# NVIDIA/cuopt

Measured on NVIDIA H100. Metric: pdlp_iterations_per_sec, higher is better.
Workload: dtype f64

## Files before the change

### cuopt_b200/csrc/pdlp_kernels.cuh

```cuda
#pragma once

#include "device_utils.cuh"
#include "spmv_bicsr.cuh"

#include <math_constants.h>

namespace cuopt_b200 {

constexpr int EW_THREADS  = 256;
static __device__ int g_l2_hints = 1;

struct pdhg_ctl_t {
  double step_size, primal_weight, tau, sigma;
  double pending_weight;
  double sum_weights;
  double interaction, norm_dx2, norm_dy2;
  double reduction_exponent, growth_exponent, primal_smoothing, dual_smoothing;
  int parity;
  int pending_avg;
  int active;
  int valid;
  int k_pdhg;
  int attempts;
  int accepted;
// ... 90 lines not shown
constexpr int DIST_MAX_PEERS        = 8;
constexpr int DIST_FLAG_XBAR        = 0 * DIST_MAX_PEERS;
constexpr int DIST_FLAG_Y           = 1 * DIST_MAX_PEERS;
constexpr int DIST_FLAG_SCALARS     = 2 * DIST_MAX_PEERS;
constexpr int DIST_FLAG_XBAR_B      = 3 * DIST_MAX_PEERS;
constexpr int DIST_FLAG_Y_B         = 4 * DIST_MAX_PEERS;
constexpr int DIST_FLAG_COUNT       = 5 * DIST_MAX_PEERS;
constexpr long long DIST_SPIN_LIMIT = 20000000000LL;
struct peer_ptrs_t {
  double* p[DIST_MAX_PEERS];
};
struct peer_flags_t {
  unsigned long long* p[DIST_MAX_PEERS];
};
__device__ __forceinline__ void st_release_sys(unsigned long long* p, unsigned long long v)
{
  asm volatile("st.release.sys.global.u64 [%0], %1;" ::"l"(p), "l"(v) : "memory");
}
__device__ __forceinline__ unsigned long long ld_acquire_sys(const unsigned long long* p)
{
  unsigned long long v;
  asm volatile("ld.acquire.sys.global.u64 %0, [%1];" : "=l"(v) : "l"(p) : "memory");
  return v;
}
__device__ __forceinline__ void peer_wait(const unsigned long long* flags, int count, unsigned long long epoch)
{
  if ((int)threadIdx.x < count) {
    const long long t0 = clock64();
    while (ld_acquire_sys(flags + threadIdx.x) < epoch) {
      __nanosleep(64);
      if (clock64() - t0 > DIST_SPIN_LIMIT) __trap();
    }
  }
  __syncthreads();
}
__device__ __forceinline__ void peer_signal_grid_done(unsigned* ticket, const peer_flags_t& flags, int world, int index,
                                                      unsigned long long epoch, int index2 = -1)
{
  __threadfence_system();
  __syncthreads();
  if (threadIdx.x != 0) return;
  const unsigned t = atomicAdd(ticket, 1u);
  if (t != gridDim.x - 1) return;
  *ticket = 0u;
  __threadfence_system();
#pragma unroll
  for (int r = 0; r < DIST_MAX_PEERS; ++r)
    if (r < world) {
      st_release_sys(flags.p[r] + index, epoch);
      if (index2 >= 0) st_release_sys(flags.p[r] + index2, epoch);
    }
}

__global__ void __launch_bounds__(EW_THREADS) k_primal_step(const pdhg_ctl_t* __restrict__ ctl,
                                                            int n,
                                                            double* __restrict__ xbuf0,
                                                            double* __restrict__ xbuf1,
                                                            const double* __restrict__ aty0,
                                                            const double* __restrict__ aty1,
                                                            const double* __restrict__ c,
                                                            const double* __restrict__ l,
                                                            const double* __restrict__ u,
                                                            double* __restrict__ sum_x,
                                                            double* __restrict__ xbar)
{
  if (!ctl->active) return;
  const int cur           = ctl->parity;
  const double* x         = cur ? xbuf1 : xbuf0;
  double* xn              = cur ? xbuf0 : xbuf1;
  const double* aty       = cur ? aty1 : aty0;
  const double tau        = ctl->tau;
  const bool pending      = ctl->pending_avg != 0;
  const double w          = ctl->pending_weight;
  const int stride        = gridDim.x * blockDim.x;
  const l2_policy_t pol   = make_l2_policies(g_l2_hints);
  for (int j = blockIdx.x * blockDim.x + threadIdx.x; j < n; j += stride) {
    const double xj = x[j];
    if (pending) sum_x[j] = sum_x[j] + w * xj;
    const double gradient = ld_stream(c + j) - aty[j];
    double next           = xj - (tau * gradient);
    next                  = fmax(fmin(next, ld_stream(u + j)), ld_stream(l + j));
    xn[j]                 = next;
    st_l2(xbar + j, next - xj + next, pol.keep);
  }
}

template <bool INIT, int NPRE, bool BCAST = false>
__global__ void __launch_bounds__(BICSR_THREADS, bicsr_min_ctas(NPRE)) k_dual_step(pdhg_ctl_t* __restrict__ ctl,
                                                                             bicsr_view_t A,
                                                                             const double* __restrict__ xbar,
                                                                             double* __restrict__ ybuf0,
                                                                             double* __restrict__ ybuf1,
                                                                             const double* __restrict__ lc,
                                                                             const double* __restrict__ uc,
                                                                             double* __restrict__ sum_y,
                                                                             double* __restrict__ part_dy2,
                                                                             const unsigned long long* xbar_flags,
                                                                             int n_xbar_flags,
                                                                             const double* __restrict__ t,
                                                                             peer_ptrs_t y_peers = peer_ptrs_t{},
                                                                             peer_flags_t flags = peer_flags_t{},
                                                                             int world = 1,
                                                                             int rank = 0,
                                                                             const int* __restrict__ send = nullptr,
                                                                             int send_stride = 0)
{
  if (!ctl->active) return;
  __shared__ double rows[BICSR_WARPS][BICSR_SLOTS];
  __shared__ double red[32];
  const unsigned long long epoch = (unsigned long long)ctl->attempts + 1ull;
  if (xbar_flags) peer_wait(xbar_flags, n_xbar_flags, (unsigned long long)ctl->attempts + 1ull);
  const int cur      = ctl->parity;
  const double* y    = cur ? ybuf1 : ybuf0;
  double* yn         = cur ? ybuf0 : ybuf1;
  const double sigma = ctl->sigma;
  const bool pending = ctl->pending_avg != 0;
  const double w     = ctl->pending_weight;
  double dy2         = 0.0;
  const l2_policy_t pol = make_l2_policies(g_l2_hints);
  struct payload_t {
    double y, lc, uc, sum, init;
  };
  auto pre_op = [&](int i) {
    payload_t p;
    p.y    = y[i];
    p.lc   = ld_stream(lc + i);
    p.uc   = ld_stream(uc + i);
    p.sum  = pending ? sum_y[i] : 0.0;
    p.init = INIT ? ld_l2(t + i, pol.stream) : 0.0;
    return p;
  };
  auto row_op = [&](int i, double s, const payload_t& p) {
    if (pending) sum_y[i] = p.sum + w * p.y;
    double next      = p.y - (sigma * s);
    const double low = next + sigma * p.lc;
    const double up  = next + sigma * p.uc;
    next             = fmax(low, fmin(up, 0.0));
    st_l2(yn + i, next, pol.keep);
    if constexpr (BCAST) {
#pragma unroll
      for (int r = 0; r < DIST_MAX_PEERS; ++r)
        if (r < world) {
          const int d = __ldg(send + (size_t)r * send_stride + i);
          if (d >= 0) y_peers.p[r][d] = next;
        }
    }
    const double d   = next - p.y;
    dy2 += d * d;
  };
  spmv_bicsr_rows<payload_t, INIT, NPRE>(A, xbar, rows[threadIdx.x >> 5], pre_op, row_op, pol.keep);
  const double tot = block_reduce(dy2, red);
  if (threadIdx.x == 0) part_dy2[blockIdx.x] = tot;
  if constexpr (BCAST) peer_signal_grid_done(&ctl->ticket[2], flags, world, DIST_FLAG_Y + rank, epoch, DIST_FLAG_Y_B + rank);
}

template <bool INIT, int NPRE>
__global__ void __launch_bounds__(BICSR_THREADS, bicsr_min_ctas(NPRE)) k_transpose_step(pdhg_ctl_t* __restrict__ ctl,
                                                                                  bicsr_view_t AT,
                                                                                  const double* __restrict__ ybuf0,
                                                                                  const double* __restrict__ ybuf1,
                                                                                  const double* __restrict__ xbuf0,
                                                                                  const double* __restrict__ xbuf1,
                                                                                  double* __restrict__ aty0,
                                                                                  double* __restrict__ aty1,
                                                                                  double* __restrict__ parts,
                                                                                  const double* __restrict__ part_dy2,
                                                                                  int n_part_dy2,
                                                                                  const double* __restrict__ t)
{
// ... 338 lines not shown
                                                                  int nloc,
                                                                  const double* __restrict__ src,
                                                                  const double* __restrict__ xbuf0,
                                                                  const double* __restrict__ xbuf1,
                                                                  double* __restrict__ aty0,
                                                                  double* __restrict__ aty1,
                                                                  double* __restrict__ parts,
                                                                  const double* __restrict__ part_dy2,
                                                                  int n_part_dy2,
                                                                  double* __restrict__ scal)
{
  if (!ctl->active) return;
  __shared__ double red[32];
  const int cur     = ctl->parity;
  const double* x   = cur ? xbuf1 : xbuf0;
  const double* xn  = cur ? xbuf0 : xbuf1;
  const double* aty = cur ? aty1 : aty0;
  double* atyn      = cur ? aty0 : aty1;
  double acc[2]     = {0.0, 0.0};
  const int stride  = gridDim.x * blockDim.x;
  for (int j = blockIdx.x * blockDim.x + threadIdx.x; j < nloc; j += stride) {
    double s = 0.0;
    s += __ldcg(src + j);
    atyn[j]        = s;
    const double d = xn[j] - x[j];
    acc[0] += d * (s - aty[j]);
    acc[1] += d * d;
  }
  if (!publish_and_elect<2>(acc, parts, &ctl->ticket[0], red)) return;
  const double interaction = gather_partials(parts, gridDim.x, red);
  const double dx2         = gather_partials(parts + gridDim.x, gridDim.x, red);
  const double dy2         = gather_partials(part_dy2, n_part_dy2, red);
  if (threadIdx.x != 0) return;
  scal[0] = interaction;
  scal[1] = dx2;
  scal[2] = dy2;
}

__global__ void k_step_rule_gather(pdhg_ctl_t* __restrict__ ctl, const double* __restrict__ scal, int n_src,
                                   const unsigned long long* wait_flags)
{
  if (!ctl->active) return;
  if (wait_flags) peer_wait(wait_flags, n_src, (unsigned long long)ctl->attempts + 1ull);
  if (threadIdx.x != 0) return;
  double interaction = 0.0, dx2 = 0.0, dy2 = 0.0;
  for (int g = 0; g < n_src; ++g) {
    interaction += __ldcg(scal + 4 * g + 0);
    dx2 += __ldcg(scal + 4 * g + 1);
    dy2 += __ldcg(scal + 4 * g + 2);
  }
  pdhg_step_rule(ctl, interaction, dx2, dy2);
}

__global__ void __launch_bounds__(BICSR_THREADS, BICSR_MIN_CTAS) k_block_pass(const pdhg_ctl_t* __restrict__ ctl,
                                                                              bicsr_view_t Ab,
                                                                              const double* __restrict__ x0,
                                                                              const double* __restrict__ x1,
                                                                              int pick_candidate,
                                                                              double* __restrict__ t,
                                                                              int first,
                                                                              const unsigned long long* wait_flags,
                                                                              int n_wait)
{
  if (!ctl->active) return;
  __shared__ double rows[BICSR_WARPS][BICSR_SLOTS];
  if (wait_flags) peer_wait(wait_flags, n_wait, (unsigned long long)ctl->attempts + 1ull);
  const double* x       = pick_candidate ? (ctl->parity ? x0 : x1) : x0;
  const l2_policy_t pol = make_l2_policies(g_l2_hints);
  struct payload_t {
    double init;
  };
  auto pre_op = [&](int r) {
    payload_t p;
    p.init = first ? 0.0 : ld_l2(t + r, pol.stream);
    return p;
  };
  auto row_op = [&](int r, double s, const payload_t&) { st_l2(t + r, s, pol.stream); };
  spmv_bicsr_rows<payload_t, true>(Ab, x, rows[threadIdx.x >> 5], pre_op, row_op, pol.keep);
}

__global__ void __launch_bounds__(EW_THREADS) k_flush_average(const pdhg_ctl_t* __restrict__ ctl,
                                                              int n,
                                                              const double* __restrict__ xbuf0,
                                                              const double* __restrict__ xbuf1,
                                                              double* __restrict__ sum_x,
                                                              int m,
                                                              const double* __restrict__ ybuf0,
                                                              const double* __restrict__ ybuf1,
                                                              double* __restrict__ sum_y)
{
  if (!ctl->pending_avg) return;
  const int cur    = ctl->parity;
  const double* x  = cur ? xbuf1 : xbuf0;
  const double* y  = cur ? ybuf1 : ybuf0;
  const double w   = ctl->pending_weight;
  const int stride = gridDim.x * blockDim.x;
  for (int j = blockIdx.x * blockDim.x + threadIdx.x; j < n; j += stride) sum_x[j] = sum_x[j] + w * x[j];
  for (int i = blockIdx.x * blockDim.x + threadIdx.x; i < m; i += stride) sum_y[i] = sum_y[i] + w * y[i];
}
__global__ void k_clear_pending(pdhg_ctl_t* ctl) { ctl->pending_avg = 0; }
__global__ void k_begin_batch(pdhg_ctl_t* ctl, int steps)
{
  ctl->target = ctl->accepted + steps;
  ctl->valid  = 0;
  ctl->active = steps > 0 ? 1 : 0;
}

__global__ void __launch_bounds__(BICSR_THREADS, BICSR_MIN_CTAS) k_spmv(bicsr_view_t A,
                                                                        const double* __restrict__ x,
                                                                        double* __restrict__ out)
{
  __shared__ double rows[BICSR_WARPS][BICSR_SLOTS];
  struct payload_t {};
  auto pre_op = [&](int) { return payload_t{}; };
  auto row_op = [&](int i, double s, const payload_t&) { out[i] = s; };
  spmv_bicsr_rows<payload_t>(A, x, rows[threadIdx.x >> 5], pre_op, row_op, make_l2_policies(g_l2_hints).keep);
}

__global__ void __launch_bounds__(BICSR_THREADS, BICSR_MIN_CTAS) k_spmv_pair(bicsr_view_t M,
                                                                             const double* __restrict__ u,
                                                                             const double* __restrict__ v,
                                                                             double* __restrict__ out_u,
                                                                             double* __restrict__ out_v,
                                                                             int first)
{
  __shared__ double rows[2][BICSR_WARPS][BICSR_SLOTS];
  auto row_op = [&](int r, double su, double sv) {
    out_u[r] = first ? su : out_u[r] + su;
    out_v[r] = first ? sv : out_v[r] + sv;
  };
  const int w = threadIdx.x >> 5;
// ... 541 lines not shown
```

### cuopt_b200/csrc/pdlp_solver.cu

```cuda
#include "pdlp_solver.hpp"

#include "dist_comm.hpp"
#include "pdlp_kernels.cuh"
#include "trust_region.cuh"

#include <math_constants.h>
#include <nvtx3/nvToolsExt.h>

#include <algorithm>
#include <chrono>
#include <cmath>
#include <cstdio>
#include <cstdlib>
#include <atomic>
#include <map>
#include <mutex>
#include <thread>
#include <string>

namespace cuopt_b200 {

namespace {

struct bicsr_dev_t {
// ... 310 lines not shown
    cudaEventSynchronize(tr_ev[last]);
    for (int i = 0; i < last; ++i) {
      float ms = 0.f;
      cudaEventElapsedTime(&ms, tr_ev[i], tr_ev[i + 1]);
      tr_acc[i] += ms;
    }
    ++tr_count;
  }
  int nslice = 0, n_pad = 0, slice_j0 = 0, slice_n = 0, grid_slice = 1;
  dvec<double> rs_buf, scal;
  dvec<unsigned long long> d_flags;
  void* xbar_peer[DIST_MAX_PEERS]  = {};
  void* scal_peer[DIST_MAX_PEERS]  = {};
  void* flag_peer[DIST_MAX_PEERS]  = {};
  bool peers_open = false;
  peer_ptrs_t p_xbar{}, p_scal{};
  peer_flags_t p_flags{};
  dvec<unsigned> d_ticket;
  dvec<pdhg_ctl_t> d_ctl;
  dvec<eval_t> d_eval;
  pdhg_ctl_t* h_ctl = nullptr;
  eval_t* h_eval    = nullptr;
  double* h_scalar  = nullptr;
  int occ_spmv = 1;
  int occ_spmv2 = 1;
  int npre_override = 0;
  dvec<double> eval_m, eval_n;
  dvec<double> part_max;
  dvec<double> part_infeas;
  bool tr_enabled = false;
  double tr_gap_reduction_last_trial = 1.0;
  int grid_tr = 1;
  dvec<double> tr_aty, tr_ax, tr_grad, tr_dir, tr_thr, tr_thr_sorted, tr_A, tr_B, tr_parts, tr_scal;
  dvec<int> tr_iota, tr_perm;
  struct tr_gap_t {
    const double *px, *py;
    double pd = 0, dd = 0, dist = 0, lower = 0, upper = 0, ngap = 0;
  };
  struct gather_blocks_t {
    int B = 1, width = 0;
    std::vector<csr_dev_t> blk;
    std::vector<csr_dev_t> unscaled;
    std::vector<int> grid;
    bool on() const { return B > 1; }
  };
  gather_blocks_t blkA, blkAT, blkATslice;
  dvec<double> t_m, t_n;
  size_t gather_block_bytes = 0;
  int n_part_dy2 = 1;
  int grid_k1 = 1, grid_k2 = 1, grid_k3 = 1, grid_n = 1, grid_m = 1, grid_misc = 1;
  long long staged_fills = 0;
  std::map<int, cudaGraphExec_t> graphs;
  bool use_graphs = true;
  cudaEvent_t ev_a = nullptr, ev_b = nullptr;

  int total_pdlp_iterations      = 0;
  bool initialised               = false;
  bool need_aty                  = true;
  bool last_restart_was_average  = false;
  bool warm_started              = false;
  double last_candidate_kkt      = 0.0, last_restart_kkt = 0.0;
  double l2_norm_b = 0.0, l2_norm_c = 0.0;
  lp_solution_t sol;
  bool finished   = false;
  double t_start  = 0.0;
  long long launches = 0;

  void close_peer_memory(bool collective)
  {
    if (!peers_open) return;
    cudaStreamSynchronize(stream);
    dist->close_peers(xbar_peer);
    dist->close_peers(scal_peer);
    dist->close_peers(flag_peer);
    dist->close_peers(yfull_peer);
    peers_open = false;
    if (collective) {
      dist->allreduce(d_scalar.data(), 1, true, stream);
      cudaStreamSynchronize(stream);
    }
  }

  ~impl_t()
  {
    if (trace.on) {
      const alloc_stats_t& a = alloc_stats();
      std::fprintf(stderr, "[cuopt-b200 trace] so far in this process: %ld cudaMalloc %.1f ms (%.2f GB), %ld cudaFree %.1f ms\n",
                   a.n_malloc, 1e3 * a.malloc_s, a.bytes * 1e-9, a.n_free, 1e3 * a.free_s);
    }
    if (dist_trace && tr_count > 0)
      std::fprintf(stderr, "[cuopt-b200 dist trace] rank %d of %d, gather transport, %ld attempts: K1 %.1f us, K2 %.1f us, K3 %.1f us, rule %.1f us "
                   "(each slot includes the wait for the peers' flags)\n", dist->rank, dist->world, tr_count,
                   1e3 * tr_acc[0] / tr_count, 1e3 * tr_acc[1] / tr_count, 1e3 * tr_acc[2] / tr_count, 1e3 * tr_acc[3] / tr_count);
    for (auto& e : tr_ev) if (e) cudaEventDestroy(e);
    if (ev_fork) cudaEventDestroy(ev_fork);
    if (ev_join) cudaEventDestroy(ev_join);
    if (comm_stream) cudaStreamDestroy(comm_stream);
    close_peer_memory(false);
    for (auto& g : graphs) cudaGraphExecDestroy(g.second);
    if (ev_a) cudaEventDestroy(ev_a);
    if (ev_b) cudaEventDestroy(ev_b);
    if (h_ctl) cudaFreeHost(h_ctl);
    if (h_eval) cudaFreeHost(h_eval);
    if (h_scalar) cudaFreeHost(h_scalar);
    if (stream) cudaStreamDestroy(stream);
  }

  int spmv_grid(const csr_dev_t& M, int npre = 1) const
  {
    const int reserve = (dist_gather && dist_send_kernel) ? send_slots : 0;
    const int wave    = std::max(1, sms * (npre > 1 ? occ_spmv2 : occ_spmv) - reserve);
    return std::max(1, std::min((M.n_blk() + BICSR_WARPS - 1) / BICSR_WARPS, wave));
  }
  int fused_npre(const csr_dev_t& M) const
  {
    if (npre_override) return npre_override > 1 ? 2 : 1;
    const bicsr_dev_t& b = M.bi_structure();
    return (b.n_std > 0 && (long long)M.rows > 40LL * b.n_std) ? 2 : 1;
  }

  void sync() { CUOPT_CUDA_TRY(cudaStreamSynchronize(stream)); }
  void check_launch() { CUOPT_CUDA_TRY(cudaGetLastError()); }

  phase_trace_t trace;
  void build(const lp_problem_t& p, const pdlp_settings_t& settings)
  {
    nvtx_range_t nvtx_scope("pdlp build: upload, transpose, block-interleaved matrices");
    trace.start(nullptr);
    p.check_representation();
    trace.mark("check_representation");
    st       = settings;
    hp       = pdlp_hyper_params_t::preset(settings.pdlp_solver_mode);
    m        = p.n_constraints;
    n        = p.n_variables;
    nnz      = p.nnz();
    maximize = p.maximize;
    if (m == 0 || nnz == 0) {
      throw lp_error(error_type_t::Success, "No constraints in the problem: PDLP can't be run");
    }
    int dev = 0;
    CUOPT_CUDA_TRY(cudaGetDevice(&dev));
    CUOPT_CUDA_TRY(cudaDeviceGetAttribute(&sms, cudaDevAttrMultiProcessorCount, dev));
    CUOPT_CUDA_TRY(cudaStreamCreateWithFlags(&stream, cudaStreamNonBlocking));
    CUOPT_CUDA_TRY(cudaEventCreate(&ev_a));
    CUOPT_CUDA_TRY(cudaEventCreate(&ev_b));
    CUOPT_CUDA_TRY(cudaMallocHost(&h_ctl, sizeof(pdhg_ctl_t)));
    CUOPT_CUDA_TRY(cudaMallocHost(&h_eval, 2 * sizeof(eval_t)));
    CUOPT_CUDA_TRY(cudaMallocHost(&h_scalar, 8 * sizeof(double)));
    if (const char* e = std::getenv("CUOPT_B200_NO_GRAPH")) use_graphs = !(e[0] == '1');
    if (const char* e = std::getenv("CUOPT_B200_L2_HINTS")) {
      const int on = e[0] != '0';
      CUOPT_CUDA_TRY(cudaMemcpyToSymbol(g_l2_hints, &on, sizeof(int)));
    }

    obj_scale  = p.objective_scaling_factor;
    obj_offset = p.objective_offset;
    if (maximize) obj_scale = -obj_scale;
    trace.stream = stream;
    trace.mark("stream + pinned control buffers");
    const long long fills0 = staged_uploader_t::get().fills();
    upload_csr(A, m, n, p.A_offsets, p.A_indices, p.A_values, stream, sms);
    trace.mark("upload A + BICSR(A)");
    transpose_to(AT, A, stream, sms);
    trace.mark("transpose + BICSR(A^T)");
    As.alias_structure_copy_values(A, stream);
    ATs.alias_structure_copy_values(AT, stream);
    const int gn = ew_grid(n, sms), gm = ew_grid(m, sms);
    upload_staged(c, p.objective_coefficients, stream);
    if (maximize) k_scale_constant<<<gn, EW_THREADS, 0, stream>>>(n, c.data(), -1.0);
    if (p.variable_lower_bounds.empty()) {
      l.resize(n);
      k_fill<<<gn, EW_THREADS, 0, stream>>>(n, l.data(), 0.0);
    } else {
      upload_staged(l, p.variable_lower_bounds, stream);
    }
    if (p.variable_upper_bounds.empty()) {
      u.resize(n);
      k_fill<<<gn, EW_THREADS, 0, stream>>>(n, u.data(), std::numeric_limits<double>::infinity());
    } else {
      upload_staged(u, p.variable_upper_bounds, stream);
    }
    if (!p.constraint_lower_bounds.empty()) {
      upload_staged(lc, p.constraint_lower_bounds, stream);
      upload_staged(uc, p.constraint_upper_bounds, stream);
    } else {
      hvec<double> hlc, huc;
      p.row_bounds(hlc, huc);
      upload_staged(lc, hlc, stream);
      upload_staged(uc, huc, stream);
      sync();
    }
    {
      dvec<int> bad(2);
      bad.zero(stream);
      k_count_crossed_bounds<<<gn, EW_THREADS, 0, stream>>>(n, l.data(), u.data(), bad.data());
      k_count_crossed_bounds<<<gm, EW_THREADS, 0, stream>>>(m, lc.data(), uc.data(), bad.data() + 1);
      check_launch();
      int h_bad[2] = {0, 0};
      CUOPT_CUDA_TRY(cudaMemcpyAsync(h_bad, bad.data(), sizeof(h_bad), cudaMemcpyDeviceToHost, stream));
      sync();
      if (h_bad[0]) throw lp_error(error_type_t::ValidationError, "Variable lower bound above upper bound");
      if (h_bad[1]) throw lp_error(error_type_t::ValidationError, "Constraint lower bound above upper bound");
// ... 550 lines not shown
      g.blk[b].cols = M.cols;
      g.blk[b].off.resize((size_t)M.rows + 1);
      offs[b] = g.blk[b].off.data();
    }
    csr_split_columns_offsets(M.rows, M.off_ptr(), M.idx_ptr(), g.width, B, offs.data(), nnz_b.data(), stream);
    for (int b = 0; b < B; ++b) {
      g.blk[b].nnz = nnz_b[b];
      g.blk[b].idx.resize((size_t)nnz_b[b]);
      g.blk[b].val.resize((size_t)nnz_b[b]);
      idxs[b] = g.blk[b].idx.data();
      vals[b] = g.blk[b].val.data();
    }
    csr_split_columns_fill(M.rows, M.off_ptr(), M.idx_ptr(), M.val.data(), g.width, B, offs.data(), idxs.data(), vals.data(),
                           stream);
    std::vector<int> hoff((size_t)M.rows + 1);
    g.grid.resize(B);
    for (int b = 0; b < B; ++b) {
      g.blk[b].off.download(hoff.data(), stream);
      sync();
      build_bicsr(g.blk[b], hoff, stream, sms);
      g.grid[b] = spmv_grid(g.blk[b]);
    }
    if (unscaled_src) {
      g.unscaled.resize(B);
      for (int b = 0; b < B; ++b) {
        csr_dev_t& U = g.unscaled[b];
        U.rows = M.rows; U.cols = M.cols; U.nnz = nnz_b[b];
        U.structure = &g.blk[b];
        U.val.resize((size_t)nnz_b[b]);
        vals[b] = U.val.data();
      }
      csr_split_columns_fill(M.rows, M.off_ptr(), M.idx_ptr(), unscaled_src->val.data(), g.width, B, offs.data(), idxs.data(),
                             vals.data(), stream);
      for (csr_dev_t& U : g.unscaled) {
        fill_bicsr_values(U, stream, sms);
        if (U.bi_structure().n_std == U.bi_structure().n_blk) {
          sync();
          U.val = dvec<double>{};
        }
      }
    }
    t.resize((size_t)M.rows);
    t.zero(stream);
  }
  void launch_block_passes(const gather_blocks_t& g, int count, const double* x0, const double* x1, int pick_candidate,
                           double* t, const unsigned long long* wait_flags, int n_wait)
  {
    for (int b = 0; b < count; ++b) {
      const csr_dev_t& M = g.blk[b];
      k_block_pass<<<g.grid[b], BICSR_THREADS, 0, stream>>>(d_ctl.data(), M.view(), x0, x1, pick_candidate, t, b == 0,
                                                            b == 0 ? wait_flags : nullptr, n_wait);
    }
  }
  void enqueue_k2(const unsigned long long* wait_flags, int n_wait, bool bcast = false,
                  const unsigned long long* wait_flags_b = nullptr)
  {
    const bool blocked  = blkA.on();
    const csr_dev_t& L  = blocked ? blkA.blk[blkA.B - 1] : hot_A();
    const int npre      = fused_npre(L);
    const int grid      = spmv_grid(L, npre);
    const double* t     = blocked ? t_m.data() : nullptr;
    const unsigned long long* wf = wait_flags_b ? wait_flags_b : (blocked ? nullptr : wait_flags);
    if (blocked) launch_block_passes(blkA, blkA.B - 1, xbar.data(), xbar.data(), 0, t_m.data(), wait_flags, n_wait);
#define CUOPT_K2(INIT, NPRE)                                                                                             \
  k_dual_step<INIT, NPRE><<<grid, BICSR_THREADS, 0, stream>>>(d_ctl.data(), L.view(), xbar.data(), ybuf[0].data(),       \
                                                              ybuf[1].data(), lcs.data(), ucs.data(), sum_y.data(),      \
                                                              part_dy2.data(), wf, n_wait, t)
#define CUOPT_K2B(INIT, NPRE)                                                                                            \
  k_dual_step<INIT, NPRE, true><<<grid, BICSR_THREADS, 0, stream>>>(d_ctl.data(), L.view(), xbar.data(), ybuf[0].data(), \
                                                                    ybuf[1].data(), lcs.data(), ucs.data(), sum_y.data(), \
                                                                    part_dy2.data(), wf, n_wait, t, p_yfull, p_flags,     \
                                                                    dist->world, dist->rank, sendY.data(), m)
    if (bcast) {
      if (blocked) { if (npre > 1) CUOPT_K2B(true, 2); else CUOPT_K2B(true, 1); }
      else { if (npre > 1) CUOPT_K2B(false, 2); else CUOPT_K2B(false, 1); }
    } else if (blocked) { if (npre > 1) CUOPT_K2(true, 2); else CUOPT_K2(true, 1); }
    else { if (npre > 1) CUOPT_K2(false, 2); else CUOPT_K2(false, 1); }
#undef CUOPT_K2B
#undef CUOPT_K2
  }
  int k2_grid() const
  {
    const csr_dev_t& L = blkA.on() ? blkA.blk[blkA.B - 1] : hot_A();
    return spmv_grid(L, fused_npre(L));
  }
  int k3_npre() const { return npre_override > 1 ? 2 : 1; }
  int k3_grid() const { return spmv_grid(blkAT.on() ? blkAT.blk[blkAT.B - 1] : ATs, k3_npre()); }
  void enqueue_k3()
  {
    const bool blocked = blkAT.on();
    const csr_dev_t& L = blocked ? blkAT.blk[blkAT.B - 1] : ATs;
    const int npre     = k3_npre();
    const int grid     = k3_grid();
    const double* t    = blocked ? t_n.data() : nullptr;
    if (blocked) launch_block_passes(blkAT, blkAT.B - 1, ybuf[0].data(), ybuf[1].data(), 1, t_n.data(), nullptr, 0);
#define CUOPT_K3(INIT, NPRE)                                                                                              \
  k_transpose_step<INIT, NPRE><<<grid, BICSR_THREADS, 0, stream>>>(d_ctl.data(), L.view(), ybuf[0].data(), ybuf[1].data(), \
                                                                   xbuf[0].data(), xbuf[1].data(), atybuf[0].data(),      \
                                                                   atybuf[1].data(), part_k3.data(), part_dy2.data(),     \
                                                                   n_part_dy2, t)
    if (blocked) { if (npre > 1) CUOPT_K3(true, 2); else CUOPT_K3(true, 1); }
    else { if (npre > 1) CUOPT_K3(false, 2); else CUOPT_K3(false, 1); }
#undef CUOPT_K3
  }
  int kernels_per_attempt() const
  {
    const int k2 = blkA.on() ? blkA.B : 1;
    if (!sharded()) return 1 + k2 + (blkAT.on() ? blkAT.B : 1);
    if (dist_gather) return 1 + k2 + (blkATslice.on() ? blkATslice.B : 1) + 1 + (dist_send_kernel ? 2 : 0);
    return 1 + k2 + (blkAT.on() ? blkAT.B : 1) + 2;
  }

  void launch_transpose_partial()
  {
    if (blkAT.on()) {
      launch_block_passes(blkAT, blkAT.B, ybuf[0].data(), ybuf[1].data(), 1, dist_buf.data(), nullptr, 0);
      return;
    }
    k_transpose_partial<<<grid_k3, BICSR_THREADS, 0, stream>>>(d_ctl.data(), ATs.view(), ybuf[0].data(), ybuf[1].data(),
                                                               dist_buf.data());
  }
  void launch_spmv(const csr_dev_t& M, const double* v, double* out)
  {
    k_spmv<<<spmv_grid(M), BICSR_THREADS, 0, stream>>>(M.view(), v, out);
  }
  int launch_spmv_pair(const csr_dev_t& M, const gather_blocks_t& g, const double* u, const double* v, double* out_u,
                       double* out_v)
  {
    const int count = g.unscaled.empty() ? 1 : (int)g.unscaled.size();
    for (int b = 0; b < count; ++b) {
// ... 21 lines not shown
      } else {
        k_primal_step_bcast<<<grid_slice, EW_THREADS, 0, stream>>>(d_ctl.data(), slice_n, x0, x1, a0, a1, cs.data() + j0,
                                                                   ls.data() + j0, us.data() + j0, sum_x.data() + j0, p_xbar,
                                                                   p_flags, G, rk, sendX.data(), nslice);
      }
      tr_tick(1);
      enqueue_k2(fl + DIST_FLAG_XBAR, G, !dist_send_kernel, fl + DIST_FLAG_XBAR_B);
      tr_tick(2);
      if (dist_send_kernel) {
        CUOPT_CUDA_TRY(cudaEventRecord(ev_fork, stream));
        CUOPT_CUDA_TRY(cudaStreamWaitEvent(comm_stream, ev_fork, 0));
        k_send_packed<<<grid_send, EW_THREADS, 0, comm_stream>>>(d_ctl.data(), ybuf[0].data(), ybuf[1].data(), 1, listY.data(),
                                                                 sendY.data(), m, planY, p_yfull, p_flags, G, rk,
                                                                 DIST_FLAG_Y, DIST_FLAG_Y_B, d_ticket.data() + 4);
        CUOPT_CUDA_TRY(cudaEventRecord(ev_join, comm_stream));
      }
      const bool blocked = blkATslice.on();
      const csr_dev_t& L = blocked ? blkATslice.blk[blkATslice.B - 1] : ATslice;
      const int grid     = spmv_grid(L, 1);
      if (blocked)
        launch_block_passes(blkATslice, blkATslice.B - 1, yfull.data(), yfull.data(), 0, t_slice.data(), fl + DIST_FLAG_Y, G);
#define CUOPT_K3S(INIT)                                                                                                     \
  k_transpose_step_slice<INIT, 1><<<grid, BICSR_THREADS, 0, stream>>>(                                                      \
    d_ctl.data(), L.view(), yfull.data(), x0, x1, a0, a1, part_k3.data(), part_dy2.data(), n_part_dy2,                      \
    blocked ? t_slice.data() : nullptr, fl + DIST_FLAG_Y_B, G, p_scal, p_flags, G, rk)
      if (blocked) CUOPT_K3S(true); else CUOPT_K3S(false);
#undef CUOPT_K3S
      tr_tick(3);
      k_step_rule_gather<<<1, 32, 0, stream>>>(d_ctl.data(), scal.data(), G, d_flags.data() + DIST_FLAG_SCALARS);
      if (dist_send_kernel) CUOPT_CUDA_TRY(cudaStreamWaitEvent(stream, ev_join, 0));
      tr_tick(4);
      tr_close(4);
      return;
    }
    k_primal_step<<<grid_slice, EW_THREADS, 0, stream>>>(d_ctl.data(), slice_n, x0, x1, a0, a1, cs.data() + j0,
                                                         ls.data() + j0, us.data() + j0, sum_x.data() + j0,
                                                         xbar.data() + j0);
    dist->allgather(xbar.data(), nslice, stream);
    enqueue_k2(nullptr, 0);
    launch_transpose_partial();
    dist->reduce_scatter(dist_buf.data(), rs_buf.data(), nslice, stream);
    k_interaction_slice<<<grid_slice, EW_THREADS, 0, stream>>>(d_ctl.data(), slice_n, rs_buf.data(), x0, x1, a0, a1,
                                                               part_k3.data(), part_dy2.data(), n_part_dy2, scal.data());
    dist->allreduce(scal.data(), 3, false, stream);
    k_step_rule_gather<<<1, 32, 0, stream>>>(d_ctl.data(), scal.data(), 1, nullptr);
  }

  void enqueue_attempt()
  {
    if (sharded()) {
      enqueue_sliced_attempt();
      return;
    }
    k_primal_step<<<grid_k1, EW_THREADS, 0, stream>>>(d_ctl.data(), n, xbuf[0].data(), xbuf[1].data(), atybuf[0].data(),
                                                      atybuf[1].data(), cs.data(), ls.data(), us.data(), sum_x.data(),
                                                      xbar.data());
    enqueue_k2(nullptr, 0);
    enqueue_k3();
  }

  void launch_attempts(int count)
  {
    if (count <= 0) return;
    launches += (long long)kernels_per_attempt() * count;
    if (!use_graphs || count == 1) {
      for (int i = 0; i < count; ++i) enqueue_attempt();
      check_launch();
      return;
    }
    auto it = graphs.find(count);
    if (it == graphs.end()) {
      cudaGraph_t g;
      CUOPT_CUDA_TRY(cudaStreamBeginCapture(stream, cudaStreamCaptureModeThreadLocal));
      for (int i = 0; i < count; ++i) enqueue_attempt();
      CUOPT_CUDA_TRY(cudaStreamEndCapture(stream, &g));
      cudaGraphExec_t ge;
      CUOPT_CUDA_TRY(cudaGraphInstantiate(&ge, g, 0));
      cudaGraphDestroy(g);
      it = graphs.emplace(count, ge).first;
    }
    CUOPT_CUDA_TRY(cudaGraphLaunch(it->second, stream));
  }

  void fetch_ctl()
  {
    CUOPT_CUDA_TRY(cudaMemcpyAsync(h_ctl, d_ctl.data(), sizeof(pdhg_ctl_t), cudaMemcpyDeviceToHost, stream));
    sync();
  }

  void run_steps(int steps)
  {
    if (steps <= 0) return;
    nvtx_range_t nvtx_scope("take_step batch (PDHG attempts up to the next major iteration)");
    CUOPT_CUDA_TRY(cudaEventRecord(ev_a, stream));
    k_begin_batch<<<1, 1, 0, stream>>>(d_ctl.data(), steps);
    if (need_aty) {
      const int cur = h_ctl->parity;
      if (blkAT.on() && !sharded()) {
        launch_block_passes(blkAT, blkAT.B, ybuf[cur].data(), ybuf[cur].data(), 0, atybuf[cur].data(), nullptr, 0);
        launches += blkAT.B;
      } else {
        launch_spmv(ATs, ybuf[cur].data(), atybuf[cur].data());
        ++launches;
      }
      if (sharded()) dist->allreduce(atybuf[cur].data(), n, false, stream);
      need_aty = false;
    }
    const int target = h_ctl->accepted + steps;
    int todo         = steps;
// ... 516 lines not shown
  : impl_(new impl_t)
{
  const double t0 = now_seconds();
  impl_->dist = dist;
  impl_->build(problem, settings);
  impl_->sol.stats.setup_seconds += now_seconds() - t0;
}
pdlp_solver_t::~pdlp_solver_t() = default;

void pdlp_solver_t::initialise() { impl_->initialise(); }
bool pdlp_solver_t::advance(int accepted_steps) { return impl_->outer_loop(accepted_steps); }
const lp_solution_t& pdlp_solver_t::solution() const { return impl_->sol; }

lp_solution_t pdlp_solver_t::run()
{
  impl_t& s        = *impl_;
  const double t0  = now_seconds();
  s.t_start        = t0;
  s.outer_loop(-1);
  s.close_peer_memory(true);
  s.sol.stats.solve_time = now_seconds() - t0;
  return s.sol;
}

double pdlp_solver_t::scalar(const std::string& name)
{
  impl_t& s = *impl_;
  s.fetch_ctl();
  const pdhg_ctl_t& k = *s.h_ctl;
  if (name == "step_size") return k.step_size;
  if (name == "primal_weight") return k.primal_weight;
  if (name == "tau") return k.tau;
  if (name == "sigma") return k.sigma;
  if (name == "sum_w") return k.sum_weights;
  if (name == "k_total") return s.total_pdlp_iterations;
  if (name == "k_pdhg") return k.attempts;
  if (name == "its_since_restart") return k.its_since_restart;
  if (name == "interaction") return k.interaction;
  if (name == "norm_dx2") return k.norm_dx2;
  if (name == "norm_dy2") return k.norm_dy2;
  if (name == "l2_norm_b") return s.l2_norm_b;
  if (name == "l2_norm_c") return s.l2_norm_c;
  if (name == "last_restart_kkt") return s.last_restart_kkt;
  if (name == "last_candidate_kkt") return s.last_candidate_kkt;
  if (name == "n_restarts") return s.sol.stats.n_restarts;
  if (name == "last_restart_was_average") return s.last_restart_was_average ? 1.0 : 0.0;
  if (name == "eval_blocks") return (double)std::max<size_t>(1, s.blkA.unscaled.size());
  if (name == "eval_blocks_t") return (double)std::max<size_t>(1, s.blkAT.unscaled.size());
  if (name == "valid") return k.valid;
  if (name == "sm_count") return s.sms;
  if (name == "occ_spmv") return s.occ_spmv;
  if (name == "occ_spmv2") return s.occ_spmv2;
  if (name == "grid_k1") return s.grid_k1;
  if (name == "grid_k2") return s.k2_grid();
  if (name == "grid_k3") return s.k3_grid();
  if (name == "grid_n") return s.grid_n;
  if (name == "grid_m") return s.grid_m;
  if (name == "k2_npre") return s.fused_npre(s.blkA.on() ? s.blkA.blk[s.blkA.B - 1] : s.hot_A());
  if (name == "n_std_a") return s.As.bi_structure().n_std;
  if (name == "n_blk_a") return s.As.bi_structure().n_blk;
  if (name == "n_std_at") return s.ATs.bi_structure().n_std;
  if (name == "n_blk_at") return s.ATs.bi_structure().n_blk;
  if (name == "staged_fills") return (double)s.staged_fills;
  if (name == "device_cache_hits") return (double)device_block_cache_t::get().hits();
  return std::nan("");
}

std::vector<double> pdlp_solver_t::vector(const std::string& name)
{
  impl_t& s = *impl_;
  s.fetch_ctl();
  const int cur         = s.h_ctl->parity;
  const dvec<double>* v = nullptr;
  if (name == "x") v = &s.xbuf[cur];
  else if (name == "y") v = &s.ybuf[cur];
  else if (name == "aty") v = &s.atybuf[cur];
  else if (name == "x_next") v = &s.xbuf[cur ^ 1];
  else if (name == "y_next") v = &s.ybuf[cur ^ 1];
  else if (name == "aty_next") v = &s.atybuf[cur ^ 1];
  else if (name == "x_bar") v = &s.xbar;
  else if (name == "sum_x") v = &s.sum_x;
  else if (name == "sum_y") v = &s.sum_y;
  else if (name == "x_avg") v = &s.x_avg;
  else if (name == "y_avg") v = &s.y_avg;
  else if (name == "row_scaling") v = &s.Dr;
  else if (name == "col_scaling") v = &s.Dc;
  else if (name == "scaled_values") v = &s.As.val;
  else if (name == "scaled_values_t") v = &s.ATs.val;
  else if (name == "scaled_c") v = &s.cs;
  else if (name == "scaled_l") v = &s.ls;
  else if (name == "scaled_u") v = &s.us;
  else if (name == "scaled_lc") v = &s.lcs;
  else if (name == "scaled_uc") v = &s.ucs;
  else if (name == "x_last_restart") v = &s.x_lr;
  else if (name == "y_last_restart") v = &s.y_lr;
  if (!v) throw lp_error(error_type_t::InvalidArgument, "unknown vector " + name);
  std::vector<double> h(v->size());
  v->download(h.data(), s.stream);
  s.sync();
  return h;
}

void pdlp_solver_t::trust_region_bounds(const double* px, const double* py, double radius, double& lower, double& upper)
{
  impl_t& s = *impl_;
  if (!s.tr_enabled) throw lp_error(error_type_t::InvalidArgument, "trust-region bounds need pdlp_solver_mode Methodical1");
  if (!s.initialised) throw lp_error(error_type_t::InvalidArgument, "trust-region bounds need an initialised session");
  if (!(radius >= 0.0)) throw lp_error(error_type_t::InvalidArgument, "trust-region radius must be >= 0");
  s.fetch_ctl();
  s.trust_region_bounds_at(px, py, radius, lower, upper);
}

kernel_profile_t pdlp_solver_t::profile_kernels(int warmup_steps, int reps)
{
  impl_t& s = *impl_;
  s.initialise();
  if (warmup_steps > 0) s.outer_loop(warmup_steps);
  kernel_profile_t out;
  out.reps = reps;
  out.grid_primal = s.grid_k1; out.grid_dual = s.grid_k2; out.grid_transpose = s.grid_k3;
  out.blocks_dual = s.blkA.B; out.blocks_transpose = s.blkAT.B;
  const double n = s.n, m = s.m, nz = s.nnz;
  out.bytes_primal_step    = 8.0 * (5 * n + 2 * n + 2 * n);
  out.bytes_dual_step      = 12.0 * nz + 4.0 * (m + 1) + 8.0 * (n + 3 * m + m + 2 * m);
  out.bytes_transpose_step = 12.0 * nz + 4.0 * (n + 1) + 8.0 * (m + n + 3 * n);
  s.need_aty = false;
  k_begin_batch<<<1, 1, 0, s.stream>>>(s.d_ctl.data(), 1 << 30);
  std::vector<cudaEvent_t> ev(4);
  for (auto& e : ev) cudaEventCreate(&e);
  double acc[3] = {0, 0, 0};
  for (int r = 0; r < reps + 3; ++r) {
    cudaEventRecord(ev[0], s.stream);
    k_primal_step<<<s.grid_k1, EW_THREADS, 0, s.stream>>>(s.d_ctl.data(), s.n, s.xbuf[0].data(), s.xbuf[1].data(),
                                                          s.atybuf[0].data(), s.atybuf[1].data(), s.cs.data(), s.ls.data(),
                                                          s.us.data(), s.sum_x.data(), s.xbar.data());
    cudaEventRecord(ev[1], s.stream);
    s.enqueue_k2(nullptr, 0);
    cudaEventRecord(ev[2], s.stream);
    s.enqueue_k3();
    cudaEventRecord(ev[3], s.stream);
    cudaEventSynchronize(ev[3]);
    if (r >= 3) {
      for (int q = 0; q < 3; ++q) {
        float ms = 0.f;
        cudaEventElapsedTime(&ms, ev[q], ev[q + 1]);
        acc[q] += ms;
      }
    }
  }
  s.check_launch();
  out.ms_primal_step    = acc[0] / reps;
  out.ms_dual_step      = acc[1] / reps;
  out.ms_transpose_step = acc[2] / reps;
  cudaEventRecord(ev[0], s.stream);
  s.launch_attempts(reps);
  cudaEventRecord(ev[1], s.stream);
  cudaEventSynchronize(ev[1]);
  float ms = 0.f;
  cudaEventElapsedTime(&ms, ev[0], ev[1]);
  out.ms_iteration = ms / reps;
  {
    dvec<double> scratch((size_t)s.n);
    for (int r = 0; r < reps + 3; ++r) {
      if (r == 3) cudaEventRecord(ev[0], s.stream);
      k_transpose_partial<<<s.grid_k3, BICSR_THREADS, 0, s.stream>>>(s.d_ctl.data(), s.ATs.view(), s.ybuf[0].data(),
                                                                    s.ybuf[1].data(), scratch.data());
    }
    cudaEventRecord(ev[1], s.stream);
    cudaEventSynchronize(ev[1]);
    cudaEventElapsedTime(&ms, ev[0], ev[1]);
    out.ms_transpose_partial      = ms / reps;
    out.ms_transpose_partial_wide = 0.0;
    s.check_launch();
  }
  for (auto& e : ev) cudaEventDestroy(e);
  s.sync();
  return out;
}

lp_solution_t solve_lp(const lp_problem_t& problem, const pdlp_settings_t& settings, dist_context_t* dist)
{
  lp_solution_t sol;
  try {
    pdlp_solver_t solver(problem, settings, dist);
    sol = solver.run();
  } catch (const lp_error& e) {
    if (e.type == error_type_t::Success) {
      sol.termination_status = termination_status_t::NumericalError;
// ... 22 lines not shown
```

### cuopt_b200/csrc/spmv_bicsr.cuh

```cuda
#pragma once

#include "device_utils.cuh"

namespace cuopt_b200 {

constexpr int BICSR_CH              = 8;
constexpr int BICSR_SLOTS           = 32 * BICSR_CH;
constexpr int BICSR_MAX_ROWS        = 256;
constexpr int BICSR_THREADS         = 256;
constexpr int BICSR_WARPS           = BICSR_THREADS / 32;
constexpr int BICSR_PAD             = 0x7fffffff;
constexpr unsigned short BICSR_EMPTY = 0xffff;
constexpr int BICSR_MIN_CTAS        = 4;
__host__ __device__ constexpr int bicsr_min_ctas(int npre) { return npre > 1 ? 3 : BICSR_MIN_CTAS; }

__host__ __device__ constexpr int bicsr_slot(int q) { return (q % BICSR_CH) * 32 + q / BICSR_CH; }

struct bicsr_view_t {
  const int2* desc;
  const unsigned short* row_slot;
  const int* idx;
  const double* val;
  int n_std, n_blk;
  const int* off;
  const int* cidx;
  const double* cval;
};

__device__ __forceinline__ void bicsr_block_row_sums(const double (&a)[BICSR_CH], const double (&g)[BICSR_CH], unsigned ends,
                                                     int lane, double* rsw)
{
  constexpr unsigned FULL = 0xffffffffu;
  double s = 0.0, head = 0.0;
  const int kf = ends ? __ffs(ends) - 1 : -1;
#pragma unroll
  for (int k = 0; k < BICSR_CH; ++k) {
    s = __dadd_rn(s, __dmul_rn(a[k], g[k]));
    const bool e = (ends >> k) & 1u;
    if (e && k != kf) rsw[k * 32 + lane] = s;
    head = (k == kf) ? s : head;
    s    = e ? 0.0 : s;
  }
  double tail  = s;
  double carry = __shfl_up_sync(FULL, tail, 1);
  if (lane == 0) carry = 0.0;
  unsigned pending = __ballot_sync(FULL, kf < 0);
  while (pending) {
    if (kf < 0) tail = carry + s;
    carry = __shfl_up_sync(FULL, tail, 1);
    if (lane == 0) carry = 0.0;
    pending &= pending << 1;
  }
  if (kf >= 0) rsw[kf * 32 + lane] = carry + head;
}

template <typename P, bool INIT = false, int NPRE = 1, typename PreOp, typename RowOp>
__device__ __forceinline__ void spmv_bicsr_rows(const bicsr_view_t& A,
                                                const double* __restrict__ x,
                                                double* rsw,
                                                PreOp& pre_op,
                                                RowOp& row_op,
                                                unsigned long long gather_policy)
{
  const int lane          = threadIdx.x & 31;
  const int gwarp         = blockIdx.x * BICSR_WARPS + (threadIdx.x >> 5);
  const int nwarps        = gridDim.x * BICSR_WARPS;
  int c[BICSR_CH];
  if (gwarp < A.n_std) {
#pragma unroll
    for (int k = 0; k < BICSR_CH; ++k) c[k] = ld_stream(A.idx + (size_t)gwarp * BICSR_SLOTS + k * 32 + lane);
  }
  for (int b = gwarp; b < A.n_std; b += nwarps) {
    const int2 d  = __ldg(A.desc + b);
    const int r0 = d.x, r1 = d.y;
    P pl[NPRE];
    unsigned short slot[NPRE];
#pragma unroll
    for (int q = 0; q < NPRE; ++q) {
      slot[q] = BICSR_EMPTY;
      if (r0 + lane + 32 * q < r1) {
        pl[q]   = pre_op(r0 + lane + 32 * q);
        slot[q] = __ldg(A.row_slot + r0 + lane + 32 * q);
      }
    }
    const size_t base = (size_t)b * BICSR_SLOTS + lane;
    double a[BICSR_CH], g[BICSR_CH];
#pragma unroll
    for (int k = 0; k < BICSR_CH; ++k) a[k] = ld_stream(A.val + base + k * 32);
#pragma unroll
    for (int k = 0; k < BICSR_CH; ++k) {
      const int col = c[k] & 0x7fffffff;
      g[k]          = col != BICSR_PAD ? ld_l2(x + col, gather_policy) : 0.0;
    }
    unsigned ends = 0;
#pragma unroll
    for (int k = 0; k < BICSR_CH; ++k) ends |= (unsigned)(c[k] < 0) << k;
    if (b + nwarps < A.n_std) {
#pragma unroll
      for (int k = 0; k < BICSR_CH; ++k) c[k] = ld_stream(A.idx + (size_t)(b + nwarps) * BICSR_SLOTS + k * 32 + lane);
    }
    bicsr_block_row_sums(a, g, ends, lane, rsw);
    __syncwarp();
#pragma unroll
    for (int q = 0; q < NPRE; ++q) {
      if (r0 + lane + 32 * q < r1) {
        double sum = slot[q] != BICSR_EMPTY ? rsw[slot[q]] : 0.0;
        if constexpr (INIT) sum = pl[q].init + sum;
        row_op(r0 + lane + 32 * q, sum, pl[q]);
      }
    }
    for (int r = r0 + 32 * NPRE + lane; r < r1; r += 32) {
      const P p2              = pre_op(r);
      const unsigned short s2 = __ldg(A.row_slot + r);
      double sum              = s2 != BICSR_EMPTY ? rsw[s2] : 0.0;
      if constexpr (INIT) sum = p2.init + sum;
      row_op(r, sum, p2);
    }
    __syncwarp();
  }
  for (int b = A.n_std + gwarp; b < A.n_blk; b += nwarps) {
    const int row = __ldg(A.desc + b).x;
    const int lo = __ldg(A.off + row), hi = __ldg(A.off + row + 1);
    P pl;
    if (lane == 0) pl = pre_op(row);
    double acc = 0.0;
    for (int e = lo + lane; e < hi; e += 32) acc += ld_stream(A.cval + e) * ld_l2(x + ld_stream(A.cidx + e), gather_policy);
    acc = warp_sum(acc);
    if (lane == 0) {
      if constexpr (INIT) acc = pl.init + acc;
      row_op(row, acc, pl);
    }
  }
}

template <typename RowOp>
__device__ __forceinline__ void spmv_bicsr_rows_pair(const bicsr_view_t& A,
                                                     const double* __restrict__ u,
                                                     const double* __restrict__ v,
                                                     double* rsw_u,
                                                     double* rsw_v,
                                                     RowOp& row_op,
// ... 104 lines not shown
```

Before: 366.2.

## Overlap primal step columns and dual averaging with blocked SpMV passes

```diff
diff --git a/cuopt_b200/csrc/pdlp_kernels.cuh b/cuopt_b200/csrc/pdlp_kernels.cuh
--- a/cuopt_b200/csrc/pdlp_kernels.cuh
+++ b/cuopt_b200/csrc/pdlp_kernels.cuh
@@ -166,6 +166,21 @@
     }
 }
 
+__device__ __forceinline__ void primal_step_column(int j, const double* __restrict__ x, double* __restrict__ xn,
+                                                   const double* __restrict__ aty, const double* __restrict__ c,
+                                                   const double* __restrict__ l, const double* __restrict__ u,
+                                                   double* __restrict__ sum_x, double* __restrict__ xbar, double tau,
+                                                   bool pending, double w, unsigned long long xbar_policy)
+{
+  const double xj = x[j];
+  if (pending) sum_x[j] = sum_x[j] + w * xj;
+  const double gradient = ld_stream(c + j) - aty[j];
+  double next           = xj - (tau * gradient);
+  next                  = fmax(fmin(next, ld_stream(u + j)), ld_stream(l + j));
+  xn[j]                 = next;
+  st_l2(xbar + j, next - xj + next, xbar_policy);
+}
+
 __global__ void __launch_bounds__(EW_THREADS) k_primal_step(const pdhg_ctl_t* __restrict__ ctl,
                                                             int n,
                                                             double* __restrict__ xbuf0,
@@ -188,18 +203,11 @@
   const double w          = ctl->pending_weight;
   const int stride        = gridDim.x * blockDim.x;
   const l2_policy_t pol   = make_l2_policies(g_l2_hints);
-  for (int j = blockIdx.x * blockDim.x + threadIdx.x; j < n; j += stride) {
-    const double xj = x[j];
-    if (pending) sum_x[j] = sum_x[j] + w * xj;
-    const double gradient = ld_stream(c + j) - aty[j];
-    double next           = xj - (tau * gradient);
-    next                  = fmax(fmin(next, ld_stream(u + j)), ld_stream(l + j));
-    xn[j]                 = next;
-    st_l2(xbar + j, next - xj + next, pol.keep);
-  }
-}
-
-template <bool INIT, int NPRE, bool BCAST = false>
+  for (int j = blockIdx.x * blockDim.x + threadIdx.x; j < n; j += stride)
+    primal_step_column(j, x, xn, aty, c, l, u, sum_x, xbar, tau, pending, w, pol.keep);
+}
+
+template <bool INIT, int NPRE, bool BCAST = false, bool AVG = true>
 __global__ void __launch_bounds__(BICSR_THREADS, bicsr_min_ctas(NPRE)) k_dual_step(pdhg_ctl_t* __restrict__ ctl,
                                                                              bicsr_view_t A,
                                                                              const double* __restrict__ xbar,
@@ -228,7 +236,7 @@
   const double* y    = cur ? ybuf1 : ybuf0;
   double* yn         = cur ? ybuf0 : ybuf1;
   const double sigma = ctl->sigma;
-  const bool pending = ctl->pending_avg != 0;
+  const bool pending = AVG && ctl->pending_avg != 0;
   const double w     = ctl->pending_weight;
   double dy2         = 0.0;
   const l2_policy_t pol = make_l2_policies(g_l2_hints);
@@ -673,6 +681,16 @@
   pdhg_step_rule(ctl, interaction, dx2, dy2);
 }
 
+struct side_step_t {
+  int n;
+  double *x0, *x1;
+  const double *aty0, *aty1, *c, *l, *u;
+  double *sum_x, *xbar;
+  int m;
+  const double *y0, *y1;
+  double* sum_y;
+};
+template <bool SIDE = false>
 __global__ void __launch_bounds__(BICSR_THREADS, BICSR_MIN_CTAS) k_block_pass(const pdhg_ctl_t* __restrict__ ctl,
                                                                               bicsr_view_t Ab,
                                                                               const double* __restrict__ x0,
@@ -681,7 +699,8 @@
                                                                               double* __restrict__ t,
                                                                               int first,
                                                                               const unsigned long long* wait_flags,
-                                                                              int n_wait)
+                                                                              int n_wait,
+                                                                              side_step_t side = side_step_t{})
 {
   if (!ctl->active) return;
   __shared__ double rows[BICSR_WARPS][BICSR_SLOTS];
@@ -697,7 +716,29 @@
     return p;
   };
   auto row_op = [&](int r, double s, const payload_t&) { st_l2(t + r, s, pol.stream); };
-  spmv_bicsr_rows<payload_t, true>(Ab, x, rows[threadIdx.x >> 5], pre_op, row_op, pol.keep);
+  if constexpr (!SIDE) {
+    spmv_bicsr_rows<payload_t, true>(Ab, x, rows[threadIdx.x >> 5], pre_op, row_op, pol.keep);
+  } else {
+    const int cur      = ctl->parity;
+    const double* xc   = cur ? side.x1 : side.x0;
+    double* xn         = cur ? side.x0 : side.x1;
+    const double* aty  = cur ? side.aty1 : side.aty0;
+    const double* y    = cur ? side.y1 : side.y0;
+    const double tau   = ctl->tau;
+    const bool pending = ctl->pending_avg != 0;
+    const double w     = ctl->pending_weight;
+    auto primal = [&](int e) {
+      if (e < side.n) primal_step_column(e, xc, xn, aty, side.c, side.l, side.u, side.sum_x, side.xbar, tau, pending, w,
+                                         pol.stream);
+    };
+    const int lane = threadIdx.x & 31;
+    auto block_op  = [&](int b) { primal(b * 32 + lane); };
+    spmv_bicsr_rows<payload_t, true>(Ab, x, rows[threadIdx.x >> 5], pre_op, row_op, pol.keep, block_op);
+    const int gtid = blockIdx.x * blockDim.x + threadIdx.x, stride = gridDim.x * blockDim.x;
+    for (int e = 32 * Ab.n_std + gtid; e < side.n; e += stride) primal(e);
+    if (pending)
+      for (int e = gtid; e < side.m; e += stride) side.sum_y[e] = side.sum_y[e] + w * y[e];
+  }
 }
 
 __global__ void __launch_bounds__(EW_THREADS) k_flush_average(const pdhg_ctl_t* __restrict__ ctl,
diff --git a/cuopt_b200/csrc/pdlp_solver.cu b/cuopt_b200/csrc/pdlp_solver.cu
--- a/cuopt_b200/csrc/pdlp_solver.cu
+++ b/cuopt_b200/csrc/pdlp_solver.cu
@@ -386,6 +386,7 @@
   long long staged_fills = 0;
   std::map<int, cudaGraphExec_t> graphs;
   bool use_graphs = true;
+  bool overlap_k1 = true;
   cudaEvent_t ev_a = nullptr, ev_b = nullptr;
 
   int total_pdlp_iterations      = 0;
@@ -482,6 +483,7 @@
     CUOPT_CUDA_TRY(cudaMallocHost(&h_eval, 2 * sizeof(eval_t)));
     CUOPT_CUDA_TRY(cudaMallocHost(&h_scalar, 8 * sizeof(double)));
     if (const char* e = std::getenv("CUOPT_B200_NO_GRAPH")) use_graphs = !(e[0] == '1');
+    if (const char* e = std::getenv("CUOPT_B200_OVERLAP_K1")) overlap_k1 = e[0] != '0';
     if (const char* e = std::getenv("CUOPT_B200_L2_HINTS")) {
       const int on = e[0] != '0';
       CUOPT_CUDA_TRY(cudaMemcpyToSymbol(g_l2_hints, &on, sizeof(int)));
@@ -1138,6 +1140,34 @@
                                                             b == 0 ? wait_flags : nullptr, n_wait);
     }
   }
+  bool overlapped() const { return overlap_k1 && blkA.on() && !sharded(); }
+  int k1_columns() const { return overlapped() ? blkA.width : n; }
+  void launch_k1()
+  {
+    k_primal_step<<<grid_k1, EW_THREADS, 0, stream>>>(d_ctl.data(), k1_columns(), xbuf[0].data(), xbuf[1].data(),
+                                                      atybuf[0].data(), atybuf[1].data(), cs.data(), ls.data(), us.data(),
+                                                      sum_x.data(), xbar.data());
+  }
+  void launch_k2_passes_with_side()
+  {
+    const int B = blkA.B, W = blkA.width, R = (m + B - 2) / (B - 1);
+    const int wave = std::max(1, sms * occ_spmv);
+    for (int b = 0; b < B - 1; ++b) {
+      const int j0 = std::min(n, (b + 1) * W), i0 = std::min(m, b * R);
+      side_step_t sd;
+      sd.n    = std::min(n, j0 + W) - j0;
+      sd.x0   = xbuf[0].data() + j0;   sd.x1   = xbuf[1].data() + j0;
+      sd.aty0 = atybuf[0].data() + j0; sd.aty1 = atybuf[1].data() + j0;
+      sd.c    = cs.data() + j0;        sd.l    = ls.data() + j0;        sd.u = us.data() + j0;
+      sd.sum_x = sum_x.data() + j0;    sd.xbar = xbar.data() + j0;
+      sd.m    = std::min(m, i0 + R) - i0;
+      sd.y0   = ybuf[0].data() + i0;   sd.y1   = ybuf[1].data() + i0;   sd.sum_y = sum_y.data() + i0;
+      const int side_ctas = (std::max(sd.n, sd.m) + BICSR_THREADS - 1) / BICSR_THREADS;
+      const int grid      = std::max(blkA.grid[b], std::min(wave, side_ctas));
+      k_block_pass<true><<<grid, BICSR_THREADS, 0, stream>>>(d_ctl.data(), blkA.blk[b].view(), xbar.data(), xbar.data(), 0,
+                                                             t_m.data(), b == 0, nullptr, 0, sd);
+    }
+  }
   void enqueue_k2(const unsigned long long* wait_flags, int n_wait, bool bcast = false,
                   const unsigned long long* wait_flags_b = nullptr)
   {
@@ -1147,11 +1177,14 @@
     const int grid      = spmv_grid(L, npre);
     const double* t     = blocked ? t_m.data() : nullptr;
     const unsigned long long* wf = wait_flags_b ? wait_flags_b : (blocked ? nullptr : wait_flags);
-    if (blocked) launch_block_passes(blkA, blkA.B - 1, xbar.data(), xbar.data(), 0, t_m.data(), wait_flags, n_wait);
-#define CUOPT_K2(INIT, NPRE)                                                                                             \
-  k_dual_step<INIT, NPRE><<<grid, BICSR_THREADS, 0, stream>>>(d_ctl.data(), L.view(), xbar.data(), ybuf[0].data(),       \
-                                                              ybuf[1].data(), lcs.data(), ucs.data(), sum_y.data(),      \
-                                                              part_dy2.data(), wf, n_wait, t)
+    const bool side     = overlapped();
+    if (side) launch_k2_passes_with_side();
+    else if (blocked) launch_block_passes(blkA, blkA.B - 1, xbar.data(), xbar.data(), 0, t_m.data(), wait_flags, n_wait);
+#define CUOPT_K2(INIT, NPRE, AVG)                                                                                     \
+  k_dual_step<INIT, NPRE, false, AVG><<<grid, BICSR_THREADS, 0, stream>>>(d_ctl.data(), L.view(), xbar.data(),            \
+                                                                          ybuf[0].data(), ybuf[1].data(), lcs.data(),      \
+                                                                          ucs.data(), sum_y.data(), part_dy2.data(), wf,   \
+                                                                          n_wait, t)
 #define CUOPT_K2B(INIT, NPRE)                                                                                            \
   k_dual_step<INIT, NPRE, true><<<grid, BICSR_THREADS, 0, stream>>>(d_ctl.data(), L.view(), xbar.data(), ybuf[0].data(), \
                                                                     ybuf[1].data(), lcs.data(), ucs.data(), sum_y.data(), \
@@ -1160,8 +1193,9 @@
     if (bcast) {
       if (blocked) { if (npre > 1) CUOPT_K2B(true, 2); else CUOPT_K2B(true, 1); }
       else { if (npre > 1) CUOPT_K2B(false, 2); else CUOPT_K2B(false, 1); }
-    } else if (blocked) { if (npre > 1) CUOPT_K2(true, 2); else CUOPT_K2(true, 1); }
-    else { if (npre > 1) CUOPT_K2(false, 2); else CUOPT_K2(false, 1); }
+    } else if (side) { if (npre > 1) CUOPT_K2(true, 2, false); else CUOPT_K2(true, 1, false); }
+    else if (blocked) { if (npre > 1) CUOPT_K2(true, 2, true); else CUOPT_K2(true, 1, true); }
+    else { if (npre > 1) CUOPT_K2(false, 2, true); else CUOPT_K2(false, 1, true); }
 #undef CUOPT_K2B
 #undef CUOPT_K2
   }
@@ -1289,9 +1323,7 @@
       enqueue_sliced_attempt();
       return;
     }
-    k_primal_step<<<grid_k1, EW_THREADS, 0, stream>>>(d_ctl.data(), n, xbuf[0].data(), xbuf[1].data(), atybuf[0].data(),
-                                                      atybuf[1].data(), cs.data(), ls.data(), us.data(), sum_x.data(),
-                                                      xbar.data());
+    launch_k1();
     enqueue_k2(nullptr, 0);
     enqueue_k3();
   }
@@ -1914,6 +1946,7 @@
   if (name == "occ_spmv") return s.occ_spmv;
   if (name == "occ_spmv2") return s.occ_spmv2;
   if (name == "grid_k1") return s.grid_k1;
+  if (name == "k1_columns") return s.k1_columns();
   if (name == "grid_k2") return s.k2_grid();
   if (name == "grid_k3") return s.k3_grid();
   if (name == "grid_n") return s.grid_n;
@@ -1983,8 +2016,10 @@
   out.grid_primal = s.grid_k1; out.grid_dual = s.grid_k2; out.grid_transpose = s.grid_k3;
   out.blocks_dual = s.blkA.B; out.blocks_transpose = s.blkAT.B;
   const double n = s.n, m = s.m, nz = s.nnz;
-  out.bytes_primal_step    = 8.0 * (5 * n + 2 * n + 2 * n);
-  out.bytes_dual_step      = 12.0 * nz + 4.0 * (m + 1) + 8.0 * (n + 3 * m + m + 2 * m);
+  const double n1 = s.k1_columns();
+  out.bytes_primal_step    = 8.0 * (5 * n1 + 2 * n1 + 2 * n1);
+  out.bytes_dual_step      = 12.0 * nz + 4.0 * (m + 1) + 8.0 * (n + 3 * m + m + 2 * m)
+                             + 8.0 * 9 * (n - n1);
   out.bytes_transpose_step = 12.0 * nz + 4.0 * (n + 1) + 8.0 * (m + n + 3 * n);
   s.need_aty = false;
   k_begin_batch<<<1, 1, 0, s.stream>>>(s.d_ctl.data(), 1 << 30);
@@ -1993,9 +2028,7 @@
   double acc[3] = {0, 0, 0};
   for (int r = 0; r < reps + 3; ++r) {
     cudaEventRecord(ev[0], s.stream);
-    k_primal_step<<<s.grid_k1, EW_THREADS, 0, s.stream>>>(s.d_ctl.data(), s.n, s.xbuf[0].data(), s.xbuf[1].data(),
-                                                          s.atybuf[0].data(), s.atybuf[1].data(), s.cs.data(), s.ls.data(),
-                                                          s.us.data(), s.sum_x.data(), s.xbar.data());
+    s.launch_k1();
     cudaEventRecord(ev[1], s.stream);
     s.enqueue_k2(nullptr, 0);
     cudaEventRecord(ev[2], s.stream);
diff --git a/cuopt_b200/csrc/spmv_bicsr.cuh b/cuopt_b200/csrc/spmv_bicsr.cuh
--- a/cuopt_b200/csrc/spmv_bicsr.cuh
+++ b/cuopt_b200/csrc/spmv_bicsr.cuh
@@ -54,13 +54,17 @@
   if (kf >= 0) rsw[kf * 32 + lane] = carry + head;
 }
 
-template <typename P, bool INIT = false, int NPRE = 1, typename PreOp, typename RowOp>
+struct no_block_op_t {
+  __device__ __forceinline__ void operator()(int) const {}
+};
+template <typename P, bool INIT = false, int NPRE = 1, typename PreOp, typename RowOp, typename BlockOp = const no_block_op_t>
 __device__ __forceinline__ void spmv_bicsr_rows(const bicsr_view_t& A,
                                                 const double* __restrict__ x,
                                                 double* rsw,
                                                 PreOp& pre_op,
                                                 RowOp& row_op,
-                                                unsigned long long gather_policy)
+                                                unsigned long long gather_policy,
+                                                BlockOp& block_op = no_block_op_t{})
 {
   const int lane          = threadIdx.x & 31;
   const int gwarp         = blockIdx.x * BICSR_WARPS + (threadIdx.x >> 5);
@@ -87,6 +91,7 @@
     double a[BICSR_CH], g[BICSR_CH];
 #pragma unroll
     for (int k = 0; k < BICSR_CH; ++k) a[k] = ld_stream(A.val + base + k * 32);
+    block_op(b);
 #pragma unroll
     for (int k = 0; k < BICSR_CH; ++k) {
       const int col = c[k] & 0x7fffffff;
```

After: 376.9 (median of 6 runs). 1.03x the previous value.
